# ExistentialRobotics/CORSAIR

Measured on AMD Instinct MI355X. Metric: end-to-end queries/sec (embed+retrieve+register), Scan2CAD chair, higher is better.
Workload: dtype f32 sparse conv + embedding / f64 RANSAC, k-NN, Chamfer, top-k / f16 MFMA bounds and shortlists (survivors recounted in f64)

## Files before the change

### corsair_amd/_lib.py

```python
from __future__ import annotations

import ctypes
import threading
import os
import re
from ctypes import POINTER, c_char_p, c_double, c_float, c_int, c_int32, c_int64, c_uint64, c_void_p

_HERE = os.path.dirname(os.path.abspath(__file__))
LIB_PATH = os.environ.get("CORSAIR_HIP_LIB") or os.path.join(_HERE, "csrc", "libcorsair_hip.so")
HEADER_PATH = os.path.join(os.path.dirname(_HERE), "include", "corsair_hip.h")

_lib = None


class CorsairHipError(RuntimeError):
    """Raised when a cs_* entry point returns a negative status (message = cs_last_error())."""


def _declare(lib):
    vp = c_void_p
    sigs = {
        "cs_last_error": (c_char_p, []),
        "cs_version": (c_int, []),
        "cs_device_count": (c_int, []),
        "cs_coordmap_create": (c_int, [vp, c_int64, c_int, vp, POINTER(vp)]),
        "cs_coordmap_stride": (c_int, [vp, c_int, vp, POINTER(vp)]),
        "cs_coordmap_pyramid": (c_int, [vp, c_int64, c_int, c_int, c_int, vp, POINTER(vp)]),
        "cs_coordmap_size": (c_int64, [vp]),
        "cs_coordmap_tensor_stride": (c_int, [vp]),
        "cs_coordmap_coords": (vp, [vp]),
        "cs_coordmap_free": (None, [vp]),
        "cs_kernelmap_build": (c_int, [vp, vp, c_int, c_int, vp, POINTER(vp)]),
        "cs_kernelmap_build_many": (c_int, [c_int, POINTER(vp), POINTER(vp), POINTER(c_int), POINTER(c_int), vp, POINTER(vp)]),
        "cs_kernelmap_num_pairs": (c_int64, [vp]),
        "cs_kernelmap_rows": (c_int64, [vp]),
        "cs_kernelmap_table": (vp, [vp]),
        "cs_kernelmap_export": (c_int64, [vp, vp, vp, vp, c_int64, vp]),
        "cs_kernelmap_free": (None, [vp]),
        "cs_conv_fwd": (c_int, [vp, c_int64, c_int64, vp, c_int, c_int, vp, c_int, vp, vp, vp,
                                c_int, c_int, vp, c_int, vp]),
        "cs_conv_wgrad": (c_int, [vp, c_int64, c_int64, vp, c_int, c_int, vp, c_int, c_int, vp, vp]),
        "cs_affine_act": (c_int, [c_int64, c_int, vp, c_int, vp, vp, vp, c_int, c_int, vp, c_int, vp]),
        "cs_row_l2_normalize": (c_int, [c_int64, c_int, vp, c_int, c_float, vp, c_int, vp]),
        "cs_segmented_max": (c_int, [c_int64, c_int, vp, c_int, vp, c_int, c_int, vp, vp]),
        "cs_instance_norm": (c_int, [c_int64, c_int, vp, c_int, vp, c_int, vp, vp, c_float, vp, c_int, vp]),
        "cs_voxelize": (c_int, [vp, POINTER(c_int64), c_int, c_double, vp, vp, POINTER(c_int64), vp]),
        "cs_voxelize_f64": (c_int, [vp, POINTER(c_int64), c_int, c_double, vp, vp, POINTER(c_int64), vp]),
        "cs_l2_topk": (c_int, [vp, c_int64, vp, c_int64, c_int, c_int, vp, vp, vp]),
        "cs_l2_topk_sq": (c_int, [vp, c_int64, vp, c_int64, c_int, c_int, vp, vp, vp]),
        "cs_knn_feat": (c_int, [vp, POINTER(c_int64), vp, POINTER(c_int64), POINTER(c_int32),
                                POINTER(c_int32), c_int, c_int, c_int, vp, vp, vp, vp, vp, vp]),
        "cs_chamfer_1dir": (c_int, [vp, POINTER(c_int64), vp, POINTER(c_int64), POINTER(c_int32),
                                    POINTER(c_int32), c_int, vp, vp, vp]),
        "cs_hausdorff_1dir": (c_int, [vp, POINTER(c_int64), vp, POINTER(c_int64), POINTER(c_int32),
                                      POINTER(c_int32), c_int, vp, vp, vp]),
        "cs_ransac_batch": (c_int, [vp, vp, POINTER(c_int64), c_int, c_double, c_int, c_int, c_double,
                                    c_uint64, vp, vp, vp, vp, vp]),
        "cs_ransac_prefilter_stats": (None, [POINTER(c_uint64), c_int]),
        "cs_knn_shortlist_stats": (None, [POINTER(c_uint64), c_int]),
        "cs_chamfer_f16_stats": (None, [POINTER(c_uint64), c_int]),
        "cs_l2_topk_stats": (None, [POINTER(c_uint64), c_int]),
        "cs_topk_catalog_create": (c_int, [vp, c_int64, c_int, vp, POINTER(vp)]),
        "cs_l2_topk_catalog": (c_int, [vp, c_int64, vp, c_int, vp, vp, c_int, vp]),
        "cs_topk_catalog_free": (None, [vp]),
        "cs_symcut_fit": (c_int, [vp, c_int, vp, POINTER(c_int64), c_int, vp, c_int,
                                  POINTER(c_int32), c_int, c_int, c_int, vp, vp, vp, vp, vp]),
        "cs_symcut_labels": (c_int, [vp, POINTER(c_int64), c_int, POINTER(c_int32), vp, vp, vp]),
        "cs_partition_by_label": (c_int, [vp, vp, c_int, vp, vp]),
        "cs_cfg_bad": (c_int, [vp, c_int, vp, c_int, vp, vp]),
        "cs_corr_assemble": (c_int, [vp, vp, vp, vp, c_int, vp, c_int, c_int64, vp, vp, vp]),
        "cs_radius_pairs": (c_int, [vp, POINTER(c_int64), vp, POINTER(c_int64), POINTER(c_int32), POINTER(c_int32),
                                    c_int, c_double, c_int, vp, vp, POINTER(vp)]),
        "cs_radius_pairs_fill": (c_int, [vp, vp, vp, vp]),
        "cs_radius_plan_free": (None, [vp]),
        "cs_sample_pairs": (c_int, [vp, POINTER(c_int64), POINTER(c_int32), POINTER(c_int32), POINTER(c_int32),
                                    POINTER(c_int32), c_int, POINTER(c_int64), vp, vp, c_int, c_uint64, c_int,
                                    c_double, c_int, vp, vp, vp, vp, vp]),
        "cs_transform_f64": (c_int, [vp, POINTER(c_int64), POINTER(c_int32), c_int, vp, vp, vp]),
        "cs_pair_loss_fwd": (c_int, [c_int, POINTER(vp), POINTER(c_int64), POINTER(c_int32), c_int, c_int,
                                     POINTER(c_int32), POINTER(c_int32), POINTER(c_int32), POINTER(c_float),
                                     POINTER(c_double), POINTER(vp), POINTER(c_int64), vp, vp, vp]),
        "cs_pair_loss_bwd": (c_int, [c_int, POINTER(vp), POINTER(c_int64), POINTER(c_int32), c_int, c_int,
                                     POINTER(c_int32), POINTER(c_int32), POINTER(c_int32), POINTER(c_float),
                                     POINTER(c_double), POINTER(vp), POINTER(c_int64), vp, POINTER(vp),
                                     POINTER(c_int32), vp]),
        "cs_hardest_negatives": (c_int, [vp, c_int, vp, POINTER(c_int64), vp, c_int, vp, POINTER(c_int64),
                                         POINTER(c_int32), POINTER(c_int32), c_int, c_int, vp, c_int64, c_double, vp, vp,
                                         vp]),
        "cs_hardest_stats": (None, [POINTER(c_uint64), c_int]),
        "cs_icp_batch": (c_int, [vp, POINTER(c_int64), vp, POINTER(c_int64), POINTER(c_int32), POINTER(c_int32), c_int, vp,
                                 c_double, c_int, c_double, c_double, vp, vp, vp, vp, vp, vp, vp, vp]),
        "cs_icp_stats": (None, [POINTER(c_uint64), c_int]),
        "cs_icp_plane_batch": (c_int, [vp, POINTER(c_int64), vp, vp, POINTER(c_int64), POINTER(c_int32), POINTER(c_int32),
                                       c_int, vp, c_double, c_int, c_double, c_double, vp, vp, vp, vp, vp, vp, vp, vp]),
        "cs_icp_plane_robust_batch": (c_int, [vp, POINTER(c_int64), vp, vp, POINTER(c_int64), POINTER(c_int32),
                                              POINTER(c_int32), c_int, vp, c_double, c_int, c_double, c_double, c_int,
                                              c_double, vp, vp, vp, vp, vp, vp, vp, vp, vp]),
        "cs_estimate_normals": (c_int, [vp, POINTER(c_int64), c_int, c_int, vp, vp]),
        "cs_estimate_normals_hybrid": (c_int, [vp, POINTER(c_int64), c_int, c_double, c_int, vp, vp]),
        "cs_normals_stats": (None, [POINTER(c_uint64), c_int]),
        "cs_prof_enable": (None, [c_int]),
        "cs_prof_reset": (None, []),
        "cs_prof_get": (c_int, [c_char_p, POINTER(c_double), POINTER(c_int64)]),
        "cs_prof_get_units": (c_int, [c_char_p, POINTER(c_double)]),
        "cs_pool_trim": (None, []),
        "cs_pool_stats": (None, [POINTER(c_uint64)]),
    }
    for name, (res, args) in sigs.items():
        fn = getattr(lib, name)
        fn.restype = res
        fn.argtypes = args
    return sigs


def header_symbols():
    with open(HEADER_PATH) as f:
        text = f.read()
    text = re.sub(r"/\*.*?\*/", "", text, flags=re.S)
    return sorted(set(re.findall(r"\b(cs_[a-z0-9_]+)\s*\(", text)))


def load():
    global _lib
# ... 87 lines not shown
```

### corsair_amd/backend.py

```python
from __future__ import annotations

import ctypes
from ctypes import c_void_p
from typing import NamedTuple, Optional

import numpy as np
import torch

from . import _lib
from ._lib import check, i32_array, i64_array, ptr, stream_ptr

KERNEL_VOLUME = 27


def _dev(t, dtype, what):
    if not isinstance(t, torch.Tensor) or not t.is_cuda:
        raise _lib.CorsairHipError(f"{what} must be a device tensor (the HIP path has no CPU fallback)")
    if t.dtype != dtype:
        raise TypeError(f"{what} must be {dtype}, got {t.dtype}")
    return t


def _rows(t, what):
    if t.dim() != 2 or t.stride(1) != 1:
# ... 484 lines not shown
        corr = corr[:corr_off[-1]]
    return IcpResult(T, T32, fitness, rmse, iters, ncorr, corr, corr_off, wfitness)


def icp_stats(reset=False):
    out = (ctypes.c_uint64 * 2)()
    _lib.load().cs_icp_stats(out, 1 if reset else 0)
    return int(out[0]), int(out[1])


def ransac_batch(src, tgt, offsets, max_corr, ransac_n=10, max_iter=100000, confidence=0.999, seed=0):
    src = _dev(src, torch.float32, "source correspondences").contiguous()
    tgt = _dev(tgt, torch.float32, "target correspondences").contiguous()
    n_prob = len(offsets) - 1
    dev = src.device
    T = torch.empty((n_prob, 4, 4), dtype=torch.float32, device=dev)
    inl = torch.empty(n_prob, dtype=torch.int32, device=dev)
    rmse = torch.empty(n_prob, dtype=torch.float64, device=dev)
    iters = torch.empty(n_prob, dtype=torch.int32, device=dev)
    check(_lib.load().cs_ransac_batch(ptr(src), ptr(tgt), i64_array(offsets), n_prob, float(max_corr),
                                      ransac_n, max_iter, float(confidence), int(seed), ptr(T),
                                      ptr(inl), ptr(rmse), ptr(iters), stream_ptr()))
    return T, inl, rmse, iters


def partition_by_label(label, d_off, n_cloud):
    label = _dev(label, torch.int32, "labels").contiguous()
    order = torch.empty(label.shape[0], dtype=torch.int64, device=label.device)
    check(_lib.load().cs_partition_by_label(ptr(label), ptr(d_off), n_cloud, ptr(order), stream_ptr()))
    return order


def cfg_bad(nn, d_first, n_cfg):
    nn = _dev(nn, torch.int32, "neighbour lists").contiguous()
    bad = torch.empty(n_cfg, dtype=torch.int32, device=nn.device)
    check(_lib.load().cs_cfg_bad(ptr(nn), nn.shape[1], ptr(d_first), n_cfg, ptr(bad), stream_ptr()))
    return bad


def corr_assemble(xyz0, xyz1, rows, nn, desc, total, max_len):
    xyz0 = _dev(xyz0, torch.float32, "query xyz").contiguous()
    xyz1 = _dev(xyz1, torch.float32, "CAD xyz").contiguous()
    nn = _dev(nn, torch.int32, "neighbour lists").contiguous()
    k = nn.shape[1]
    dev = xyz0.device
    src = torch.empty((total * k, 3), dtype=torch.float32, device=dev)
    tgt = torch.empty((total * k, 3), dtype=torch.float32, device=dev)
    d_desc = torch.from_numpy(np.ascontiguousarray(desc, dtype=np.int64)).to(dev, non_blocking=True)
    check(_lib.load().cs_corr_assemble(ptr(xyz0), ptr(xyz1), ptr(rows) if rows is not None else None, ptr(nn), k,
                                       ptr(d_desc), len(desc), int(max_len), ptr(src), ptr(tgt), stream_ptr()))
    return src, tgt


def symcut_fit(feat, xyz, offsets, anchors, Ks, n_nn=50, n_init=10, max_iter=300):
    feat = _dev(feat, torch.float32, "features").contiguous()
    xyz = _dev(xyz, torch.float32, "xyz").contiguous()
    anchors = _dev(anchors, torch.int32, "anchors").contiguous()
    nc, na = anchors.shape
    dev = feat.device
    centers = torch.empty((nc, na, 4, 3), dtype=torch.float64, device=dev)
    counts = torch.empty((nc, na, 4), dtype=torch.int32, device=dev)
    mcd = torch.empty((nc, na), dtype=torch.float64, device=dev)
    mer = torch.empty((nc, na), dtype=torch.float64, device=dev)
    check(_lib.load().cs_symcut_fit(ptr(feat), feat.shape[1], ptr(xyz), i64_array(offsets), nc,
                                    ptr(anchors), na, i32_array(Ks), n_nn, n_init, max_iter,
                                    ptr(centers), ptr(counts), ptr(mcd), ptr(mer), stream_ptr()))
    return centers, counts, mcd, mer


def symcut_labels(xyz, offsets, Ks, sel_centers):
    xyz = _dev(xyz, torch.float32, "xyz").contiguous()
    sel_centers = _dev(sel_centers, torch.float64, "centres").contiguous()
    labels = torch.empty(xyz.shape[0], dtype=torch.int32, device=xyz.device)
    check(_lib.load().cs_symcut_labels(ptr(xyz), i64_array(offsets), len(Ks), i32_array(Ks),
                                       ptr(sel_centers), ptr(labels), stream_ptr()))
    return labels


class RadiusPlan:

    def __init__(self, handle, keep):
        self._h = c_void_p(handle)
        self._keep = keep

    def fill(self, row_ptr, total):
        idx = torch.empty(max(int(total), 1), dtype=torch.int32, device=row_ptr.device)
        check(_lib.load().cs_radius_pairs_fill(self._h, ptr(row_ptr), ptr(idx), stream_ptr()))
        return idx[:int(total)]

    def __del__(self):
        try:
            if self._h:
                _lib.load().cs_radius_plan_free(self._h)
                self._h = None
        except Exception:
            pass


def radius_pairs_begin(src, soff, tgt, toff, src_seg=None, tgt_seg=None, radius=0.03, k=None):
    src = _dev(src, torch.float64, "source points").contiguous()
    tgt = _dev(tgt, torch.float64, "target points").contiguous()
    if src_seg is None:
        src_seg = list(range(len(soff) - 1))
        tgt_seg = list(range(len(toff) - 1))
    if len(src_seg) != len(tgt_seg):
        raise ValueError("radius_pairs: src_seg and tgt_seg differ in length")
# ... 100 lines not shown
```

### corsair_amd/csrc/sympose.hip

```cpp
#include "common.h"

namespace cs {

__global__ __launch_bounds__(256) void k_partition_by_label(const int32_t* __restrict__ label,
                                                            const int64_t* __restrict__ off,
                                                            int64_t* __restrict__ order) {
  __shared__ int hist[8];
  __shared__ int base[8];
  __shared__ int wcnt[4][8];
  const int c = blockIdx.x;
  const int64_t r0 = off[c], r1 = off[c + 1];
  const int tid = threadIdx.x, lane = tid & 63, wave = tid >> 6;
  if (tid < 8) hist[tid] = 0;
  __syncthreads();
  for (int64_t r = r0 + tid; r < r1; r += 256) {
    int l = label[r];
    l = l < 0 ? 0 : (l > 7 ? 7 : l);
    atomicAdd(&hist[l], 1);
  }
  __syncthreads();
  if (tid == 0) {
    int run = 0;
    for (int l = 0; l < 8; ++l) {
      base[l] = run;
// ... 14 lines not shown
      const unsigned long long m = __ballot(l == q);
      if (l == q) my_rank = __popcll(m & ((1ULL << lane) - 1ULL));
      if (lane == 0) wcnt[wave][q] = __popcll(m);
    }
    __syncthreads();
    if (l >= 0) {
      int pos = base[l] + my_rank;
      for (int w = 0; w < wave; ++w) pos += wcnt[w][l];
      order[r0 + pos] = r;
    }
    __syncthreads();
    if (tid < 8) base[tid] += wcnt[0][tid] + wcnt[1][tid] + wcnt[2][tid] + wcnt[3][tid];
    __syncthreads();
  }
}

struct CorrDesc {
  int64_t q_first, n_first, t_first, len, out_first;
};
__global__ __launch_bounds__(256) void k_corr_assemble(const float* __restrict__ xyz0, const float* __restrict__ xyz1,
                                                       const int64_t* __restrict__ rows, const int32_t* __restrict__ nn,
                                                       int k, const CorrDesc* __restrict__ desc,
                                                       float* __restrict__ src, float* __restrict__ tgt) {
  const CorrDesc d = desc[blockIdx.y];
  for (int64_t e = (int64_t)blockIdx.x * 256 + threadIdx.x; e < d.len * k; e += (int64_t)gridDim.x * 256) {
    const int64_t i = e / k;
    const int nb = (int)(e - i * k);
    const int64_t q = rows ? rows[d.q_first + i] : d.q_first + i;
    const int32_t nbv = nn[(d.n_first + i) * k + nb];
    const int64_t t = d.t_first + (nbv < 0 ? 0 : nbv);
    const int64_t o = (d.out_first * k + e) * 3;
    src[o] = xyz0[q * 3];
    src[o + 1] = xyz0[q * 3 + 1];
    src[o + 2] = xyz0[q * 3 + 2];
    tgt[o] = xyz1[t * 3];
    tgt[o + 1] = xyz1[t * 3 + 1];
    tgt[o + 2] = xyz1[t * 3 + 2];
  }
}

__global__ __launch_bounds__(256) void k_cfg_bad(const int32_t* __restrict__ nn, int k, const int64_t* __restrict__ first,
                                                 int32_t* __restrict__ bad) {
  const int j = blockIdx.y;
  const int64_t a = first[j] * k, b = first[j + 1] * k;
  int any = 0;
  for (int64_t e = a + (int64_t)blockIdx.x * 256 + threadIdx.x; e < b; e += (int64_t)gridDim.x * 256) any |= nn[e] < 0;
  if (__any(any) && (threadIdx.x & 63) == 0) atomicOr(&bad[j], 1);
}
__global__ void k_zero_i32(int32_t* p, int n) {
  const int i = blockIdx.x * blockDim.x + threadIdx.x;
  if (i < n) p[i] = 0;
}

}

using namespace cs;

extern "C" {

int cs_partition_by_label(const int32_t* d_label, const int64_t* d_off, int n_cloud, int64_t* d_order, void* stream) {
  CS_REQUIRE(n_cloud >= 0 && (n_cloud == 0 || (d_label && d_off && d_order)), CS_ERR_INVALID,
             "cs_partition_by_label: bad argument");
  if (n_cloud == 0) return CS_OK;
  hipLaunchKernelGGL(k_partition_by_label, dim3((unsigned)n_cloud), dim3(256), 0, (hipStream_t)stream, d_label, d_off,
                     d_order);
  CS_LAUNCH_CHECK();
  return CS_OK;
}

int cs_corr_assemble(const float* d_xyz0, const float* d_xyz1, const int64_t* d_rows, const int32_t* d_nn, int k,
                     const int64_t* d_desc, int n_cfg, int64_t max_len, float* d_src, float* d_tgt, void* stream) {
  CS_REQUIRE(k >= 1 && n_cfg >= 0 && max_len >= 0, CS_ERR_INVALID, "cs_corr_assemble: bad argument");
  if (n_cfg == 0 || max_len == 0) return CS_OK;
  CS_REQUIRE(d_xyz0 && d_xyz1 && d_nn && d_desc && d_src && d_tgt, CS_ERR_INVALID, "cs_corr_assemble: NULL tensor");
  unsigned gx = (unsigned)ceil_div(max_len * k, 256);
  if (gx > 64) gx = 64;
  hipLaunchKernelGGL(k_corr_assemble, dim3(gx, (unsigned)n_cfg), dim3(256), 0, (hipStream_t)stream, d_xyz0, d_xyz1, d_rows,
                     d_nn, k, reinterpret_cast<const CorrDesc*>(d_desc), d_src, d_tgt);
  CS_LAUNCH_CHECK();
  return CS_OK;
}

int cs_cfg_bad(const int32_t* d_nn, int k, const int64_t* d_first, int n_cfg, int32_t* d_bad, void* stream) {
  CS_REQUIRE(k >= 1 && n_cfg >= 0, CS_ERR_INVALID, "cs_cfg_bad: bad argument");
  if (n_cfg == 0) return CS_OK;
  CS_REQUIRE(d_nn && d_first && d_bad, CS_ERR_INVALID, "cs_cfg_bad: NULL tensor");
  hipStream_t s = (hipStream_t)stream;
  hipLaunchKernelGGL(k_zero_i32, dim3((unsigned)ceil_div(n_cfg, 256)), dim3(256), 0, s, d_bad, n_cfg);
  hipLaunchKernelGGL(k_cfg_bad, dim3(16, (unsigned)n_cfg), dim3(256), 0, s, d_nn, k, d_first, d_bad);
  CS_LAUNCH_CHECK();
  return CS_OK;
}

}
```

### corsair_amd/registration.py

```python
from __future__ import annotations

import os
from dataclasses import dataclass

import numpy as np
import torch

from . import _helper
from . import backend as B
from ._lib import to_host

ANCHOR_KEY = 0x5A11C0DE



@dataclass
class SymPoseResult:
    T_best: torch.Tensor
    cd_best: torch.Tensor
    T_ransac: torch.Tensor
    cd_ransac: torch.Tensor
    ok: np.ndarray
    iters: torch.Tensor
    n_problems: int
# ... 31 lines not shown
    valid = (min_cdist > gate[0]) & (gate[1] > max_err) & (std < 100)
    if not valid.any():
        return None
    a = int(np.argmin(np.where(valid, std, np.inf)))
    c = centers[a]
    out = np.zeros((4, 3), np.float64)
    if K == 2:
        out[:2] = c[:2]
        return out
    d = np.linalg.norm(c[0][None, :] - c[1:4], axis=1)
    rank = np.argsort(d, kind="stable")
    out[:] = c[[0, rank[0] + 1, rank[2] + 1, rank[1] + 1]]
    return out


def gate_and_order_batch(centers, counts, min_cdist, max_err, n, Ks, cand, gate=GATE_REFERENCE):
    P = centers.shape[0]
    sel = np.zeros((P, 4, 3), np.float64)
    ok = np.zeros(P, dtype=bool)
    n = np.asarray(n, dtype=np.float64)
    Ks = np.asarray(Ks)
    cand = np.asarray(cand, dtype=np.int64)
    for K in (2, 4):
        idx = cand[Ks[cand] == K]
        if idx.size == 0:
            continue
        ratios = counts[idx][:, :, :K].astype(np.float64) / n[idx][:, None, None]
        std = np.sqrt(np.var(ratios, axis=2))
        valid = (min_cdist[idx] > gate[0]) & (gate[1] > max_err[idx]) & (std < 100)
        has = valid.any(axis=1)
        a = np.argmin(np.where(valid, std, np.inf), axis=1)
        c = centers[idx, a]
        out = np.zeros((idx.size, 4, 3), np.float64)
        if K == 2:
            out[:, :2] = c[:, :2]
        else:
            d = np.linalg.norm(c[:, 0:1] - c[:, 1:4], axis=2)
            rank = np.argsort(d, axis=1, kind="stable")
            order = np.stack([np.zeros(idx.size, np.int64), rank[:, 0] + 1, rank[:, 2] + 1, rank[:, 1] + 1], 1)
            out = np.take_along_axis(c, order[:, :, None], axis=1)
        sel[idx[has]] = out[has]
        ok[idx[has]] = True
    return sel, ok


def part_configs(K, pos_sym):
    cfgs = [[(i + s) % K for i in range(K)] for s in range(K)]
    if pos_sym >= 2:
        mirror = [0, 3, 2, 1]
        cfgs += [[mirror[(i + s) % 4] for i in range(4)] for s in range(4)]
    return cfgs


def sym_pose_batch(baseF, xyz0, off0, posF, xyz1, off1, pos_syms, k_nn=5, max_corr=0.20, seed=0,
                   anchor_ids=None, n_anchor=100, max_iter=100000, confidence=0.999,
                   use_symmetry=True, force_gate=False, query_anchors=None, icp_max_iter=0, icp_max_dist=None,
                   icp_estimation="point", icp_normal_k=16, normals1=None, icp_normal_radius=None, icp_kernel="l2",
                   icp_kernel_scale=None):
    if icp_kernel not in B.ICP_KERNELS:
        raise ValueError("sym_pose_batch: icp_kernel must be one of %s, got %r" % (sorted(B.ICP_KERNELS), icp_kernel))
    if icp_kernel != "l2" and icp_estimation != "plane":
        raise ValueError("sym_pose_batch: icp_kernel %r needs icp_estimation = 'plane'" % (icp_kernel,))
    if icp_max_iter > 0 and icp_kernel != "l2" and not (icp_kernel_scale is not None and icp_kernel_scale > 0):
        raise ValueError("sym_pose_batch: icp_kernel %r needs a positive icp_kernel_scale" % (icp_kernel,))
    if icp_estimation not in ("point", "plane"):
        raise ValueError("sym_pose_batch: icp_estimation must be 'point' or 'plane', got %r" % (icp_estimation,))
    if icp_normal_radius is not None and not (0 < icp_normal_radius < float("inf")):
        raise ValueError("sym_pose_batch: icp_normal_radius must be positive and finite (None = k-NN), got %r"
                         % (icp_normal_radius,))
    if icp_max_iter > 0 and not (icp_max_dist is not None and icp_max_dist > 0):
        raise ValueError("sym_pose_batch: icp_max_iter > 0 needs a positive icp_max_dist")
    dev = baseF.device
    P = len(off0) - 1
    off0 = [int(v) for v in off0]
    off1 = [int(v) for v in off1]
    n0 = [off0[p + 1] - off0[p] for p in range(P)]
    n1 = [off1[p + 1] - off1[p] for p in range(P)]
    k = k_nn

    short = [p for p in range(P) if n0[p] > 0 and n1[p] < k]
    if short:
        raise IndexError("sym_pose_batch: CAD cloud of pair %d has %d voxels, fewer than k_nn = %d (the reference's "
                         "find_kcorr fails on such a pair too)" % (short[0], n1[short[0]], k))
    nn = B.knn_feat(baseF, off0, posF, off1, k)
    desc_v = np.asarray([[off0[p], off0[p], off1[p], n0[p], off0[p]] for p in range(P)], dtype=np.int64).reshape(P, 5)
    v_src, v_tgt = B.corr_assemble(xyz0, xyz1, None, nn, desc_v, off0[-1], max(n0) if P else 0)
    corr_src = [v_src]
    corr_tgt = [v_tgt]
    prob_len = [n0[p] * k for p in range(P)]
    prob_pair = list(range(P))
    prob_cfg = [None] * P
    ok = np.zeros(P, dtype=bool)
    vanilla = None
    if use_symmetry and dev.type == "cuda" and os.environ.get("CORSAIR_SPLIT_RANSAC", "1") != "0":
        v_offs = np.concatenate([[0], np.cumsum(prob_len)]).tolist()
        for t in (v_src, v_tgt):
            t.record_stream(_helper.stream(dev))
        vanilla = _helper.submit(dev, lambda: B.ransac_batch(v_src, v_tgt, v_offs, max_corr, 10, max_iter,
                                                            confidence, seed))

    try:
        if use_symmetry:
            Ks = [4 if int(pos_syms[p]) >= 2 else 2 for p in range(P)]
            if anchor_ids is None:
                anchor_ids = [(2 * p, 2 * p + 1) for p in range(P)]
            anc0 = query_anchors if query_anchors is not None else \
                [draw_anchors(n0[p], n_anchor, anchor_ids[p][0]) for p in range(P)]
            anc1 = [draw_anchors(n1[p], n_anchor, anchor_ids[p][1]) for p in range(P)]
            cand = [p for p in range(P) if anc0[p] is not None and anc1[p] is not None]
            sel0 = np.zeros((P, 4, 3))
            sel1 = np.zeros((P, 4, 3))
            if cand:
                def anchors_of(anc):
                    return np.stack([anc[p] if anc[p] is not None else np.zeros(n_anchor, np.int32) for p in range(P)])

                a_all = torch.from_numpy(np.concatenate([anchors_of(anc0), anchors_of(anc1)])).to(dev)
                off_all = off0 + [off0[-1] + o for o in off1[1:]]
                c, cnt, mcd, mer = B.symcut_fit(torch.cat([baseF, posF]), torch.cat([xyz0, xyz1]), off_all, a_all,
                                                Ks + Ks, 50, 10, 300)
                c, cnt, mcd, mer = to_host(c, cnt, mcd, mer)
                c0, cnt0, mcd0, mer0 = c[:P], cnt[:P], mcd[:P], mer[:P]
                c1, cnt1, mcd1, mer1 = c[P:], cnt[P:], mcd[P:], mer[P:]
                gate = GATE_ANY if force_gate else GATE_REFERENCE
                g0, ok0 = gate_and_order_batch(c0, cnt0, mcd0, mer0, n0, Ks, cand, gate)
                g1, ok1 = gate_and_order_batch(c1, cnt1, mcd1, mer1, n1, Ks, cand, gate)
                ok = ok0 & ok1
                sel0[ok], sel1[ok] = g0[ok], g1[ok]
            good = [p for p in range(P) if ok[p]]
            if good:
                lab0 = B.symcut_labels(xyz0, off0, Ks, torch.from_numpy(sel0).to(dev))
                lab1 = B.symcut_labels(xyz1, off1, Ks, torch.from_numpy(sel1).to(dev))
                qseg, tseg, perms, cfg_pair = [], [], [], []
                for p in good:
                    for cfg in part_configs(Ks[p], int(pos_syms[p])):
                        qseg.append(p)
                        tseg.append(p)
                        perms.append(cfg + [-3] * (8 - len(cfg)))
                        cfg_pair.append(p)
                lens = np.asarray([n0[p] for p in cfg_pair], dtype=np.int64)
                row_start = np.concatenate([[0], np.cumsum(lens)])
                n_cfg = len(cfg_pair)
                host_blk = np.concatenate([np.asarray(off0, np.int64), row_start,
                                           np.asarray(perms, np.int32).reshape(-1).view(np.int64)])
                dev_blk = torch.from_numpy(host_blk).to(dev)
                off0_t = dev_blk[:P + 1]
                first_t = dev_blk[P + 1:P + 2 + n_cfg]
                perm_t = dev_blk[P + 2 + n_cfg:].view(torch.int32).view(n_cfg, 8)
                sorted_rows = B.partition_by_label(lab0, off0_t, P)
                nn_cfg = B.knn_feat(baseF[sorted_rows], off0, posF, off1, k, qseg=qseg, tseg=tseg,
                                    qlabel=lab0[sorted_rows].contiguous(), tlabel=lab1, perm=perm_t)
                bad = to_host(B.cfg_bad(nn_cfg, first_t, n_cfg))[0] > 0
                keep = [j for j in range(n_cfg) if not bad[j]]
                if keep:
                    out_first = np.concatenate([[0], np.cumsum(lens[keep])])
                    desc = np.asarray([[off0[cfg_pair[j]], row_start[j], off1[cfg_pair[j]], lens[j], out_first[i]]
                                       for i, j in enumerate(keep)], dtype=np.int64)
                    s_src, s_tgt = B.corr_assemble(xyz0, xyz1, sorted_rows, nn_cfg, desc, int(out_first[-1]),
                                                   int(lens[keep].max()))
                    corr_src.append(s_src)
                    corr_tgt.append(s_tgt)
                    for j in keep:
                        prob_len.append(n0[cfg_pair[j]] * k)
                        prob_pair.append(cfg_pair[j])
                        prob_cfg.append([c for c in perms[j] if c >= 0])
    except BaseException:
        if vanilla is not None:
            try:
                vanilla.result()
            except Exception:
                pass
        raise

    if vanilla is None:
        src = corr_src[0] if len(corr_src) == 1 else torch.cat(corr_src)
        tgt = corr_tgt[0] if len(corr_tgt) == 1 else torch.cat(corr_tgt)
        offs = np.concatenate([[0], np.cumsum(prob_len)]).tolist()
        T, inl, rmse, iters = B.ransac_batch(src, tgt, offs, max_corr, 10, max_iter, confidence, seed)
    else:
        parts = []
        if len(corr_src) > 1:
            offs = np.concatenate([[0], np.cumsum(prob_len[P:])]).tolist()
            parts = [B.ransac_batch(corr_src[1], corr_tgt[1], offs, max_corr, 10, max_iter, confidence, seed)]
        first = vanilla.result()
        cur = torch.cuda.current_stream(dev)
        for t in first:
            t.record_stream(cur)
        T, inl, rmse, iters = (torch.cat([a] + [q[i] for q in parts]) for i, a in enumerate(first))

    cd = B.chamfer_1dir(xyz0, off0, xyz1, off1, prob_pair, prob_pair, T)

    cd_h = to_host(cd)[0]
    pair_h = np.asarray(prob_pair)
    best = np.arange(P)
    for j in range(P, len(pair_h)):
        p = pair_h[j]
        if cd_h[best[p]] > cd_h[j]:
            best[p] = j
    best_t = torch.from_numpy(best).to(dev)
    res = SymPoseResult(T_best=T[best_t], cd_best=cd[best_t], T_ransac=T[:P], cd_ransac=cd[:P],
                        ok=ok, iters=iters, n_problems=len(prob_pair), T_all=T, cd_all=cd, inliers=inl,
                        prob_pair=prob_pair, prob_cfg=prob_cfg, best=best)

    if icp_max_iter > 0:
        pairs = list(range(P))
        nrm = None
        if icp_estimation == "plane":
            nrm = normals1 if normals1 is not None else B.estimate_normals(xyz1, off1, icp_normal_k, icp_normal_radius)
        r = B.icp_batch(xyz0, off0, xyz1, off1, pairs, pairs, res.T_best, icp_max_dist, icp_max_iter, tgt_normals=nrm,
                        kernel=icp_kernel, kernel_scale=icp_kernel_scale)
        res.T_icp, res.icp_fitness, res.icp_rmse, res.icp_iters = r.T32, r.fitness, r.rmse, r.iters
        res.icp_wfitness = r.wfitness
        res.cd_icp = B.chamfer_1dir(xyz0, off0, xyz1, off1, pairs, pairs, r.T32)
    return res
```

### include/corsair_hip.h

```cpp
#ifndef CORSAIR_HIP_H
#define CORSAIR_HIP_H

#include <stdint.h>

#ifdef __cplusplus
extern "C" {
#endif

#define CS_OK 0
#define CS_ERR_INVALID (-1)
#define CS_ERR_HIP (-2)
#define CS_ERR_RANGE (-3)
#define CS_ERR_DUPLICATE (-4)
#define CS_ERR_UNSUPPORTED (-5)
#define CS_ERR_INTERNAL (-6)

typedef struct cs_coordmap cs_coordmap;
typedef struct cs_kernelmap cs_kernelmap;

const char* cs_last_error(void);
int cs_version(void);
int cs_device_count(void);

int cs_coordmap_create(const int32_t* d_coords, int64_t n, int tensor_stride, void* stream,
// ... 39 lines not shown
                     const float* d_weight, const float* d_bias, float eps, float* d_out, int ld_out,
                     void* stream);

int cs_voxelize(const float* d_xyz, const int64_t* h_offsets, int n_seg, double voxel_size,
                int64_t* d_keep_idx, int32_t* d_grid, int64_t* h_out_offsets, void* stream);
int cs_voxelize_f64(const double* d_xyz, const int64_t* h_offsets, int n_seg, double voxel_size,
                    int64_t* d_keep_idx, int32_t* d_grid, int64_t* h_out_offsets, void* stream);

int cs_l2_topk(const float* d_q, int64_t nq, const float* d_x, int64_t nx, int d, int k,
               int64_t* d_idx, double* d_dist, void* stream);
int cs_l2_topk_sq(const float* d_q, int64_t nq, const float* d_x, int64_t nx, int d, int k, int64_t* d_idx,
                  double* d_dist2, void* stream);
void cs_l2_topk_stats(uint64_t out[2], int reset);
typedef struct cs_topk_catalog cs_topk_catalog;
int cs_topk_catalog_create(const float* d_x, int64_t nx, int d, void* stream, cs_topk_catalog** out);
int cs_l2_topk_catalog(const float* d_q, int64_t nq, const cs_topk_catalog* catalog, int k, int64_t* d_idx,
                       double* d_dist, int squared, void* stream);
void cs_topk_catalog_free(cs_topk_catalog* catalog);

int cs_knn_feat(const float* d_qf, const int64_t* h_qoff, const float* d_tf,
                const int64_t* h_toff, const int32_t* h_qseg, const int32_t* h_tseg, int n_prob,
                int dim, int k, const int32_t* d_qlabel, const int32_t* d_tlabel,
                const int32_t* d_perm, int32_t* d_idx, double* d_dist, void* stream);

void cs_knn_shortlist_stats(uint64_t out[2], int reset);

void cs_chamfer_f16_stats(uint64_t out[2], int reset);
int cs_chamfer_1dir(const float* d_src, const int64_t* h_soff, const float* d_tgt,
                    const int64_t* h_toff, const int32_t* h_src_seg, const int32_t* h_tgt_seg,
                    int n_prob, const float* d_T, double* d_out, void* stream);

int cs_hausdorff_1dir(const float* d_src, const int64_t* h_soff, const float* d_tgt,
                      const int64_t* h_toff, const int32_t* h_src_seg, const int32_t* h_tgt_seg,
                      int n_prob, const float* d_T, double* d_out, void* stream);

int cs_ransac_batch(const float* d_src, const float* d_tgt, const int64_t* h_off, int n_prob,
                    double max_corr, int ransac_n, int max_iter, double confidence, uint64_t seed,
                    float* d_T, int32_t* d_inliers, double* d_rmse, int32_t* d_iters,
                    void* stream);
void cs_ransac_prefilter_stats(uint64_t out[5], int reset);

int cs_symcut_fit(const float* d_feat, int dim, const float* d_xyz, const int64_t* h_off,
                  int n_cloud, const int32_t* d_anchor, int n_anchor, const int32_t* h_K,
                  int n_nn, int n_init, int max_iter, double* d_centers,
                  int32_t* d_counts, double* d_min_center_dist, double* d_max_error,
                  void* stream);
int cs_symcut_labels(const float* d_xyz, const int64_t* h_off, int n_cloud, const int32_t* h_K,
                     const double* d_sel_centers, int32_t* d_labels, void* stream);

int cs_partition_by_label(const int32_t* d_label, const int64_t* d_off, int n_cloud, int64_t* d_order, void* stream);
int cs_cfg_bad(const int32_t* d_nn, int k, const int64_t* d_first, int n_cfg, int32_t* d_bad, void* stream);
int cs_corr_assemble(const float* d_xyz0, const float* d_xyz1, const int64_t* d_rows, const int32_t* d_nn, int k,
                     const int64_t* d_desc, int n_cfg, int64_t max_len, float* d_src, float* d_tgt, void* stream);

typedef struct cs_radius_plan cs_radius_plan;
int cs_radius_pairs(const double* d_src, const int64_t* h_soff, const double* d_tgt, const int64_t* h_toff,
                    const int32_t* h_src_seg, const int32_t* h_tgt_seg, int n_prob, double radius, int k_max,
                    int64_t* d_row_ptr, void* stream, cs_radius_plan** plan);
int cs_radius_pairs_fill(const cs_radius_plan* plan, const int64_t* d_row_ptr, int32_t* d_tgt_idx, void* stream);
void cs_radius_plan_free(cs_radius_plan* plan);

int cs_sample_pairs(const float* d_xyz, const int64_t* h_off, const int32_t* h_base_seg, const int32_t* h_pos_seg,
                    const int32_t* h_neg_seg, const int32_t* h_slot, int n_prob, const int64_t* h_row_base,
                    const int64_t* d_row_ptr, const int32_t* d_tgt_idx, int lists, uint64_t seed, int round,
                    double radius, int sample, int32_t* d_pip, int32_t* d_pin, int32_t* d_nin, int32_t* d_counts,
                    void* stream);

int cs_transform_f64(const float* d_xyz, const int64_t* h_off, const int32_t* h_seg, int n_prob, const double* d_T,
                     double* d_out, void* stream);

#define CS_PAIR_LOSS_MAX_TERMS 8
#define CS_PAIR_PULL 0
#define CS_PAIR_PUSH 1
int cs_pair_loss_fwd(int n_mat, const float* const* d_mat, const int64_t* h_rows, const int32_t* h_ld, int C,
                     int n_term, const int32_t* h_a, const int32_t* h_b, const int32_t* h_kind, const float* h_margin,
                     const double* h_weight, const int32_t* const* d_pairs, const int64_t* h_npairs,
                     double* d_term_loss, float* d_total, void* stream);
int cs_pair_loss_bwd(int n_mat, const float* const* d_mat, const int64_t* h_rows, const int32_t* h_ld, int C,
                     int n_term, const int32_t* h_a, const int32_t* h_b, const int32_t* h_kind, const float* h_margin,
                     const double* h_weight, const int32_t* const* d_pairs, const int64_t* h_npairs,
                     const float* d_grad_up, float* const* d_grad, const int32_t* h_ld_grad, void* stream);

int cs_hardest_negatives(const float* d_qf, int ld_q, const float* d_qxyz, const int64_t* h_qoff, const float* d_tf,
                         int ld_t, const float* d_txyz, const int64_t* h_toff, const int32_t* h_qseg,
                         const int32_t* h_tseg, int n_prob, int C, const int32_t* d_anchor, int64_t A, double radius,
                         int32_t* d_idx, double* d_dist, void* stream);
void cs_hardest_stats(uint64_t out[2], int reset);

int cs_icp_batch(const float* d_src, const int64_t* h_soff, const float* d_tgt, const int64_t* h_toff,
                 const int32_t* h_src_seg, const int32_t* h_tgt_seg, int n_prob, const float* d_T0, double max_dist,
                 int max_iter, double relative_fitness, double relative_rmse, double* d_T, float* d_T32,
                 double* d_fitness, double* d_rmse, int32_t* d_iters, int32_t* d_ncorr, int32_t* d_corr, void* stream);
void cs_icp_stats(uint64_t out[2], int reset);

int cs_icp_plane_batch(const float* d_src, const int64_t* h_soff, const float* d_tgt, const float* d_tgt_normal,
                       const int64_t* h_toff, const int32_t* h_src_seg, const int32_t* h_tgt_seg, int n_prob,
                       const float* d_T0, double max_dist, int max_iter, double relative_fitness, double relative_rmse,
                       double* d_T, float* d_T32, double* d_fitness, double* d_rmse, int32_t* d_iters, int32_t* d_ncorr,
                       int32_t* d_corr, void* stream);

#define CS_ICP_KERNEL_L2 0
#define CS_ICP_KERNEL_HUBER 1
#define CS_ICP_KERNEL_CAUCHY 2
#define CS_ICP_KERNEL_TUKEY 3
int cs_icp_plane_robust_batch(const float* d_src, const int64_t* h_soff, const float* d_tgt, const float* d_tgt_normal,
                              const int64_t* h_toff, const int32_t* h_src_seg, const int32_t* h_tgt_seg, int n_prob,
// ... 24 lines not shown
```

Before: 2087.

## Derive vanilla and config correspondences from a shared per-part k-NN table

When symmetry is used, the code now runs a single k-NN per (query part, CAD part) pair and keeps the distances. The vanilla whole-cloud top-k is rebuilt by merging the per-part sorted lists, and each part-permutation config's correspondences are read straight from that table. This replaces the separate vanilla k-NN and the per-config k-NN passes, and all correspondences go into one buffer so the final concatenation is skipped. In exchange it adds a merge kernel that recomputes f64 feature distances on ties, and split-RANSAC overlap is now off by default on this path.

Result: no change. 2116 (median of 4 runs) (+1.4%).

```diff
diff --git a/corsair_amd/_lib.py b/corsair_amd/_lib.py
--- a/corsair_amd/_lib.py
+++ b/corsair_amd/_lib.py
@@ -69,6 +69,8 @@
         "cs_partition_by_label": (c_int, [vp, vp, c_int, vp, vp]),
         "cs_cfg_bad": (c_int, [vp, c_int, vp, c_int, vp, vp]),
         "cs_corr_assemble": (c_int, [vp, vp, vp, vp, c_int, vp, c_int, c_int64, vp, vp, vp]),
+        "cs_parts_cfg_bad": (c_int, [vp, vp, c_int, vp, c_int, vp, vp]),
+        "cs_corr_from_parts": (c_int, [vp, vp, vp, vp, c_int, vp, vp, vp, vp, c_int, vp, c_int, c_int64, vp, vp, vp]),
         "cs_radius_pairs": (c_int, [vp, POINTER(c_int64), vp, POINTER(c_int64), POINTER(c_int32), POINTER(c_int32),
                                     c_int, c_double, c_int, vp, vp, POINTER(vp)]),
         "cs_radius_pairs_fill": (c_int, [vp, vp, vp, vp]),
diff --git a/corsair_amd/backend.py b/corsair_amd/backend.py
--- a/corsair_amd/backend.py
+++ b/corsair_amd/backend.py
@@ -560,6 +560,30 @@
     return src, tgt
 
 
+def parts_cfg_bad(qlabel, pt_idx, d_desc, n_cfg):
+    qlabel = _dev(qlabel, torch.int32, "query labels").contiguous()
+    pt_idx = _dev(pt_idx, torch.int32, "part table").contiguous()
+    bad = torch.empty(n_cfg, dtype=torch.int32, device=pt_idx.device)
+    check(_lib.load().cs_parts_cfg_bad(ptr(qlabel), ptr(pt_idx), pt_idx.shape[1], ptr(d_desc), n_cfg, ptr(bad),
+                                       stream_ptr()))
+    return bad
+
+
+def corr_from_parts(xyz0, xyz1, qf, tf, rows, qlabel, pt_idx, pt_dist, d_desc, n_desc, max_len, src, tgt):
+    xyz0 = _dev(xyz0, torch.float32, "query xyz").contiguous()
+    xyz1 = _dev(xyz1, torch.float32, "CAD xyz").contiguous()
+    qf = _dev(qf, torch.float32, "query features").contiguous()
+    tf = _dev(tf, torch.float32, "CAD features").contiguous()
+    qlabel = _dev(qlabel, torch.int32, "query labels").contiguous()
+    pt_idx = _dev(pt_idx, torch.int32, "part table").contiguous()
+    pt_dist = _dev(pt_dist, torch.float64, "part table distances").contiguous()
+    if qf.shape[1] != tf.shape[1] or not src.is_contiguous() or not tgt.is_contiguous():
+        raise ValueError("corr_from_parts: feature dimensions differ or outputs are not contiguous")
+    check(_lib.load().cs_corr_from_parts(ptr(xyz0), ptr(xyz1), ptr(qf), ptr(tf), qf.shape[1], ptr(rows), ptr(qlabel),
+                                         ptr(pt_idx), ptr(pt_dist), pt_idx.shape[1], ptr(d_desc), n_desc, int(max_len),
+                                         ptr(src), ptr(tgt), stream_ptr()))
+
+
 def symcut_fit(feat, xyz, offsets, anchors, Ks, n_nn=50, n_init=10, max_iter=300):
     feat = _dev(feat, torch.float32, "features").contiguous()
     xyz = _dev(xyz, torch.float32, "xyz").contiguous()
diff --git a/corsair_amd/csrc/sympose.hip b/corsair_amd/csrc/sympose.hip
--- a/corsair_amd/csrc/sympose.hip
+++ b/corsair_amd/csrc/sympose.hip
@@ -90,6 +90,107 @@
   if (i < n) p[i] = 0;
 }
 
+struct PartDesc {
+  int64_t q_first, pt_first, t_first, len, out_first, n_part, cfg;
+};
+
+__device__ __forceinline__ double chain_dist(const float* __restrict__ a, const float* __restrict__ b, int dim) {
+  double d = 0.0;
+  for (int c = 0; c < dim; ++c) {
+    const double diff = (double)a[c] - (double)b[c];
+    d = fma(diff, diff, d);
+  }
+  return d;
+}
+
+__device__ __forceinline__ int part_of(const PartDesc& d, int label) {
+  return (label >= 0 && label < (int)d.n_part) ? (int)((d.cfg >> (4 * label)) & 15) : -1;
+}
+
+__device__ int merged_entry(const PartDesc& d, const int32_t* __restrict__ pt_idx, const double* __restrict__ pt_dist,
+                            int k, int64_t i, int nb, const float* __restrict__ q, const float* __restrict__ tf, int dim) {
+  unsigned heads = 0;
+  int32_t taken = -1;
+  for (int step = 0; step <= nb; ++step) {
+    int bj = -1;
+    int32_t bi = -1;
+    double bd = 0.0;
+    for (int j = 0; j < (int)d.n_part; ++j) {
+      const int h = (heads >> (4 * j)) & 15;
+      if (h >= k) continue;
+      const int64_t e = (d.pt_first + j * d.len + i) * k + h;
+      const int32_t ci = pt_idx[e];
+      if (ci < 0) continue;
+      const double cd = pt_dist[e];
+      bool better = bj < 0 || cd < bd;
+      if (bj >= 0 && cd == bd) {
+        const double xc = chain_dist(q, tf + (d.t_first + ci) * dim, dim);
+        const double xb = chain_dist(q, tf + (d.t_first + bi) * dim, dim);
+        better = xc < xb || (xc == xb && ci < bi);
+      }
+      if (better) {
+        bj = j;
+        bi = ci;
+        bd = cd;
+      }
+    }
+    if (bj < 0) return -1;
+    heads += 1u << (4 * bj);
+    taken = bi;
+  }
+  return taken;
+}
+
+__global__ __launch_bounds__(256) void k_corr_from_parts(const float* __restrict__ xyz0, const float* __restrict__ xyz1,
+                                                         const float* __restrict__ qf, const float* __restrict__ tf,
+                                                         int dim, const int64_t* __restrict__ rows,
+                                                         const int32_t* __restrict__ qlabel,
+                                                         const int32_t* __restrict__ pt_idx,
+                                                         const double* __restrict__ pt_dist, int k,
+                                                         const PartDesc* __restrict__ desc, float* __restrict__ src,
+                                                         float* __restrict__ tgt) {
+  const PartDesc d = desc[blockIdx.y];
+  for (int64_t e = (int64_t)blockIdx.x * 256 + threadIdx.x; e < d.len * k; e += (int64_t)gridDim.x * 256) {
+    const int64_t i = e / k;
+    const int nb = (int)(e - i * k);
+    int64_t q;
+    int32_t nbv;
+    if (d.cfg < 0) {
+      q = d.q_first + i;
+      nbv = merged_entry(d, pt_idx, pt_dist, k, i, nb, qf + q * dim, tf, dim);
+    } else {
+      q = rows[d.q_first + i];
+      const int part = part_of(d, qlabel[q]);
+      nbv = part >= 0 ? pt_idx[(d.pt_first + part * d.len + (q - d.q_first)) * k + nb] : -1;
+    }
+    const int64_t t = d.t_first + (nbv < 0 ? 0 : nbv);
+    const int64_t o = (d.out_first * k + e) * 3;
+    src[o] = xyz0[q * 3];
+    src[o + 1] = xyz0[q * 3 + 1];
+    src[o + 2] = xyz0[q * 3 + 2];
+    tgt[o] = xyz1[t * 3];
+    tgt[o + 1] = xyz1[t * 3 + 1];
+    tgt[o + 2] = xyz1[t * 3 + 2];
+  }
+}
+
+__global__ __launch_bounds__(256) void k_parts_cfg_bad(const int32_t* __restrict__ qlabel,
+                                                       const int32_t* __restrict__ pt_idx, int k,
+                                                       const PartDesc* __restrict__ desc, int32_t* __restrict__ bad) {
+  const PartDesc d = desc[blockIdx.y];
+  int any = 0;
+  for (int64_t i = (int64_t)blockIdx.x * 256 + threadIdx.x; i < d.len; i += (int64_t)gridDim.x * 256) {
+    const int part = part_of(d, qlabel[d.q_first + i]);
+    if (part < 0) {
+      any = 1;
+    } else {
+      const int32_t* l = pt_idx + (d.pt_first + part * d.len + i) * k;
+      for (int nb = 0; nb < k; ++nb) any |= l[nb] < 0;
+    }
+  }
+  if (__any(any) && (threadIdx.x & 63) == 0) atomicOr(&bad[blockIdx.y], 1);
+}
+
 }
 
 using namespace cs;
@@ -130,4 +231,36 @@
   return CS_OK;
 }
 
-}
+int cs_parts_cfg_bad(const int32_t* d_qlabel, const int32_t* d_pt_idx, int k, const int64_t* d_desc, int n_cfg,
+                     int32_t* d_bad, void* stream) {
+  CS_REQUIRE(k >= 1 && k <= 15 && n_cfg >= 0, CS_ERR_INVALID, "cs_parts_cfg_bad: bad argument");
+  if (n_cfg == 0) return CS_OK;
+  CS_REQUIRE(d_qlabel && d_pt_idx && d_desc && d_bad, CS_ERR_INVALID, "cs_parts_cfg_bad: NULL tensor");
+  hipStream_t s = (hipStream_t)stream;
+  hipLaunchKernelGGL(k_zero_i32, dim3((unsigned)ceil_div(n_cfg, 256)), dim3(256), 0, s, d_bad, n_cfg);
+  hipLaunchKernelGGL(k_parts_cfg_bad, dim3(16, (unsigned)n_cfg), dim3(256), 0, s, d_qlabel, d_pt_idx, k,
+                     reinterpret_cast<const PartDesc*>(d_desc), d_bad);
+  CS_LAUNCH_CHECK();
+  return CS_OK;
+}
+
+int cs_corr_from_parts(const float* d_xyz0, const float* d_xyz1, const float* d_qf, const float* d_tf, int dim,
+                       const int64_t* d_rows, const int32_t* d_qlabel, const int32_t* d_pt_idx,
+                       const double* d_pt_dist, int k, const int64_t* d_desc, int n_desc, int64_t max_len,
+                       float* d_src, float* d_tgt, void* stream) {
+  CS_REQUIRE(k >= 1 && k <= 15 && dim >= 1 && n_desc >= 0 && max_len >= 0, CS_ERR_INVALID,
+             "cs_corr_from_parts: bad argument");
+  if (n_desc == 0 || max_len == 0) return CS_OK;
+  CS_REQUIRE(d_xyz0 && d_xyz1 && d_qf && d_tf && d_rows && d_qlabel && d_pt_idx && d_pt_dist && d_desc && d_src &&
+                 d_tgt,
+             CS_ERR_INVALID, "cs_corr_from_parts: NULL tensor");
+  unsigned gx = (unsigned)ceil_div(max_len * k, 256);
+  if (gx > 64) gx = 64;
+  hipLaunchKernelGGL(k_corr_from_parts, dim3(gx, (unsigned)n_desc), dim3(256), 0, (hipStream_t)stream, d_xyz0, d_xyz1,
+                     d_qf, d_tf, dim, d_rows, d_qlabel, d_pt_idx, d_pt_dist, k, reinterpret_cast<const PartDesc*>(d_desc),
+                     d_src, d_tgt);
+  CS_LAUNCH_CHECK();
+  return CS_OK;
+}
+
+}
diff --git a/corsair_amd/registration.py b/corsair_amd/registration.py
--- a/corsair_amd/registration.py
+++ b/corsair_amd/registration.py
@@ -107,6 +107,54 @@
     return cfgs
 
 
+def corr_from_part_table(baseF, xyz0, off0, posF, xyz1, off1, lab0, lab1, n_part, cfg_pair, perms, k, on_vanilla=None):
+    dev = baseF.device
+    P = len(off0) - 1
+    n0 = [off0[p + 1] - off0[p] for p in range(P)]
+    n_cfg = len(cfg_pair)
+    lens = np.asarray([n0[p] for p in cfg_pair], dtype=np.int64)
+    pt_seg = [p for p in range(P) for _ in range(n_part[p])]
+    pt_perm = [[j] * 8 for p in range(P) for j in range(n_part[p])]
+    pt_first = np.concatenate([[0], np.cumsum([n_part[p] * n0[p] for p in range(P)])])
+    out_first = np.concatenate([[0], np.cumsum(lens)])
+    nib = [sum(c << (4 * l) for l, c in enumerate(cf) if c >= 0) for cf in perms]
+    desc = np.asarray([[off0[p], pt_first[p], off1[p], n0[p], off0[p], n_part[p], -1] for p in range(P)] +
+                      [[off0[p], pt_first[p], off1[p], n0[p], off0[-1] + out_first[j], n_part[p], nib[j]]
+                       for j, p in enumerate(cfg_pair)], dtype=np.int64).reshape(P + n_cfg, 7)
+    host_blk = np.concatenate([np.asarray(off0, np.int64), desc.reshape(-1),
+                               np.asarray(pt_perm, np.int32).reshape(-1).view(np.int64)])
+    dev_blk = torch.from_numpy(host_blk).to(dev)
+    off0_t = dev_blk[:P + 1]
+    desc_t = dev_blk[P + 1:P + 1 + desc.size].view(P + n_cfg, 7)
+    perm_t = dev_blk[P + 1 + desc.size:].view(torch.int32).view(len(pt_seg), 8)
+    sorted_rows = B.partition_by_label(lab0, off0_t, P)
+    pt_idx, pt_dist = B.knn_feat(baseF, off0, posF, off1, k, qseg=pt_seg, tseg=pt_seg, qlabel=lab0, tlabel=lab1,
+                                 perm=perm_t, return_distance=True)
+    bad_t = B.parts_cfg_bad(lab0, pt_idx, desc_t[P:], n_cfg) if n_cfg else None
+    total = off0[-1] + int(out_first[-1])
+    src_all = torch.empty((total * k, 3), dtype=torch.float32, device=dev)
+    tgt_all = torch.empty((total * k, 3), dtype=torch.float32, device=dev)
+    B.corr_from_parts(xyz0, xyz1, baseF, posF, sorted_rows, lab0, pt_idx, pt_dist, desc_t[:P], P, max(n0), src_all,
+                      tgt_all)
+    if on_vanilla is not None:
+        on_vanilla(src_all[:off0[-1] * k], tgt_all[:off0[-1] * k])
+    bad = to_host(bad_t)[0] > 0 if n_cfg else np.zeros(0, dtype=bool)
+    keep = [j for j in range(n_cfg) if not bad[j]]
+    if not keep:
+        total = off0[-1]
+    else:
+        desc_k = desc_t[P:]
+        if len(keep) < n_cfg:
+            out_k = np.concatenate([[0], np.cumsum(lens[keep])])
+            desc_h = desc[P:][keep].copy()
+            desc_h[:, 4] = off0[-1] + out_k[:-1]
+            desc_k = torch.from_numpy(desc_h).to(dev, non_blocking=True)
+            total = off0[-1] + int(out_k[-1])
+        B.corr_from_parts(xyz0, xyz1, baseF, posF, sorted_rows, lab0, pt_idx, pt_dist, desc_k, len(keep),
+                          int(lens[keep].max()), src_all, tgt_all)
+    return src_all[:total * k], tgt_all[:total * k], keep
+
+
 def sym_pose_batch(baseF, xyz0, off0, posF, xyz1, off1, pos_syms, k_nn=5, max_corr=0.20, seed=0,
                    anchor_ids=None, n_anchor=100, max_iter=100000, confidence=0.999,
                    use_symmetry=True, force_gate=False, query_anchors=None, icp_max_iter=0, icp_max_dist=None,
@@ -137,22 +185,36 @@
     if short:
         raise IndexError("sym_pose_batch: CAD cloud of pair %d has %d voxels, fewer than k_nn = %d (the reference's "
                          "find_kcorr fails on such a pair too)" % (short[0], n1[short[0]], k))
-    nn = B.knn_feat(baseF, off0, posF, off1, k)
-    desc_v = np.asarray([[off0[p], off0[p], off1[p], n0[p], off0[p]] for p in range(P)], dtype=np.int64).reshape(P, 5)
-    v_src, v_tgt = B.corr_assemble(xyz0, xyz1, None, nn, desc_v, off0[-1], max(n0) if P else 0)
-    corr_src = [v_src]
-    corr_tgt = [v_tgt]
+    part_table = use_symmetry and os.environ.get("CORSAIR_PART_TABLE", "1") != "0"
+    split = use_symmetry and dev.type == "cuda" and \
+        os.environ.get("CORSAIR_SPLIT_RANSAC", "0" if part_table else "1") != "0"
+    corr_src, corr_tgt = [], []
     prob_len = [n0[p] * k for p in range(P)]
     prob_pair = list(range(P))
     prob_cfg = [None] * P
     ok = np.zeros(P, dtype=bool)
     vanilla = None
-    if use_symmetry and dev.type == "cuda" and os.environ.get("CORSAIR_SPLIT_RANSAC", "1") != "0":
-        v_offs = np.concatenate([[0], np.cumsum(prob_len)]).tolist()
+    one_buffer = None
+
+    def submit_vanilla(v_src, v_tgt):
+        corr_src.append(v_src)
+        corr_tgt.append(v_tgt)
+        if not split:
+            return None
+        v_offs = np.concatenate([[0], np.cumsum(prob_len[:P])]).tolist()
         for t in (v_src, v_tgt):
             t.record_stream(_helper.stream(dev))
-        vanilla = _helper.submit(dev, lambda: B.ransac_batch(v_src, v_tgt, v_offs, max_corr, 10, max_iter,
-                                                            confidence, seed))
+        return _helper.submit(dev, lambda: B.ransac_batch(v_src, v_tgt, v_offs, max_corr, 10, max_iter,
+                                                          confidence, seed))
+
+    def vanilla_search():
+        nn = B.knn_feat(baseF, off0, posF, off1, k)
+        desc_v = np.asarray([[off0[p], off0[p], off1[p], n0[p], off0[p]] for p in range(P)],
+                            dtype=np.int64).reshape(P, 5)
+        return submit_vanilla(*B.corr_assemble(xyz0, xyz1, None, nn, desc_v, off0[-1], max(n0) if P else 0))
+
+    if not part_table:
+        vanilla = vanilla_search()
 
     try:
         if use_symmetry:
@@ -182,19 +244,39 @@
                 ok = ok0 & ok1
                 sel0[ok], sel1[ok] = g0[ok], g1[ok]
             good = [p for p in range(P) if ok[p]]
+            if part_table and not good:
+                vanilla = vanilla_search()
             if good:
                 lab0 = B.symcut_labels(xyz0, off0, Ks, torch.from_numpy(sel0).to(dev))
                 lab1 = B.symcut_labels(xyz1, off1, Ks, torch.from_numpy(sel1).to(dev))
-                qseg, tseg, perms, cfg_pair = [], [], [], []
+                perms, cfg_pair = [], []
                 for p in good:
                     for cfg in part_configs(Ks[p], int(pos_syms[p])):
-                        qseg.append(p)
-                        tseg.append(p)
                         perms.append(cfg + [-3] * (8 - len(cfg)))
                         cfg_pair.append(p)
+                n_cfg = len(cfg_pair)
                 lens = np.asarray([n0[p] for p in cfg_pair], dtype=np.int64)
+            if good and part_table:
+                n_part = [Ks[p] if ok[p] else 1 for p in range(P)]
+
+                def on_vanilla(v_src, v_tgt):
+                    nonlocal vanilla
+                    vanilla = submit_vanilla(v_src, v_tgt)
+
+                src_all, tgt_all, keep = corr_from_part_table(baseF, xyz0, off0, posF, xyz1, off1, lab0, lab1, n_part,
+                                                              cfg_pair, perms, k, on_vanilla)
+                one_buffer = (src_all, tgt_all)
+                if keep:
+                    nv = off0[-1] * k
+                    corr_src.append(src_all[nv:])
+                    corr_tgt.append(tgt_all[nv:])
+                    for j in keep:
+                        prob_len.append(n0[cfg_pair[j]] * k)
+                        prob_pair.append(cfg_pair[j])
+                        prob_cfg.append([c for c in perms[j] if c >= 0])
+            elif good:
+                qseg = tseg = cfg_pair
                 row_start = np.concatenate([[0], np.cumsum(lens)])
-                n_cfg = len(cfg_pair)
                 host_blk = np.concatenate([np.asarray(off0, np.int64), row_start,
                                            np.asarray(perms, np.int32).reshape(-1).view(np.int64)])
                 dev_blk = torch.from_numpy(host_blk).to(dev)
@@ -227,8 +309,11 @@
         raise
 
     if vanilla is None:
-        src = corr_src[0] if len(corr_src) == 1 else torch.cat(corr_src)
-        tgt = corr_tgt[0] if len(corr_tgt) == 1 else torch.cat(corr_tgt)
+        if one_buffer is not None:
+            src, tgt = one_buffer
+        else:
+            src = corr_src[0] if len(corr_src) == 1 else torch.cat(corr_src)
+            tgt = corr_tgt[0] if len(corr_tgt) == 1 else torch.cat(corr_tgt)
         offs = np.concatenate([[0], np.cumsum(prob_len)]).tolist()
         T, inl, rmse, iters = B.ransac_batch(src, tgt, offs, max_corr, 10, max_iter, confidence, seed)
     else:
diff --git a/include/corsair_hip.h b/include/corsair_hip.h
--- a/include/corsair_hip.h
+++ b/include/corsair_hip.h
@@ -115,6 +115,12 @@
 int cs_cfg_bad(const int32_t* d_nn, int k, const int64_t* d_first, int n_cfg, int32_t* d_bad, void* stream);
 int cs_corr_assemble(const float* d_xyz0, const float* d_xyz1, const int64_t* d_rows, const int32_t* d_nn, int k,
                      const int64_t* d_desc, int n_cfg, int64_t max_len, float* d_src, float* d_tgt, void* stream);
+int cs_parts_cfg_bad(const int32_t* d_qlabel, const int32_t* d_pt_idx, int k, const int64_t* d_desc, int n_cfg,
+                     int32_t* d_bad, void* stream);
+int cs_corr_from_parts(const float* d_xyz0, const float* d_xyz1, const float* d_qf, const float* d_tf, int dim,
+                       const int64_t* d_rows, const int32_t* d_qlabel, const int32_t* d_pt_idx,
+                       const double* d_pt_dist, int k, const int64_t* d_desc, int n_desc, int64_t max_len,
+                       float* d_src, float* d_tgt, void* stream);
 
 typedef struct cs_radius_plan cs_radius_plan;
 int cs_radius_pairs(const double* d_src, const int64_t* h_soff, const double* d_tgt, const int64_t* h_toff,
```
